# leggedrobotics/delora

Hardware: AMD Instinct MI355X
Metric: training scan-pairs/sec, KITTI 64x2048 range images (higher is better)
Workload: dtype f32; 1 GPU; KITTI-shaped 64x2048, batch=8 pairs/GPU, raw scans of ~141k points (ragged, raster order), steps rotate over 8 distinct HBM-resident batches, online normals, ResNet pose CNN (11.9M params, identity-pretrained state), Adam; BASELINE configs[1]; global_batch=8, parallelism=dp1, cnn=fp32, cnn_impl=hip trunk: fp32 MFMA, fused Winograd F(2x2,3x3) + direct implicit GEMM, channels_last=False, hip_graph=False, distinct_batches=8, priming_steps=8

## Files before the change

### delora_amd/csrc/heads.hip

```cpp
#include "common.h"

#define HD_MAXB 16

struct HeadsP {
  const float *fc_w, *fc_b;
  const float *r1_w, *r1_b;
  const float *r3_w, *r3_b;
  const float *t1_w, *t1_b;
  const float *t3_w, *t3_b;
};

__device__ __forceinline__ float hd_act(float v, int act) { return act == 1 ? dl_tanh(v) : (act == 2 ? (v < 0.f ? 0.f : v) : v); }
__device__ __forceinline__ float hd_dact(float a, int act) { return act == 1 ? 1.f - a * a : (act == 2 ? (a > 0.f ? 1.f : 0.f) : 1.f); }

__global__ __launch_bounds__(256) void k_heads_rows(const float* __restrict__ x, int B, int K, const float* __restrict__ w0, const float* __restrict__ b0,
                                                    const float* __restrict__ w1, const float* __restrict__ b1, int rows, int nmat, int act,
                                                    int KC, const float* __restrict__ pre_scale ,
                                                    float* __restrict__ y ) {
  extern __shared__ float sx[];
  const int wave = threadIdx.x >> 6, lane = threadIdx.x & 63;
  const int gr = min(blockIdx.x * 4 + wave, rows * nmat - 1);
  const int m = gr / rows, r = gr % rows;
  const float* wr = (m == 0 ? w0 : w1) + (size_t)r * K;
  float acc[HD_MAXB];
#pragma unroll
  for (int b = 0; b < HD_MAXB; ++b) acc[b] = 0.f;
  for (int k0 = 0; k0 < K; k0 += KC) {
    const int kn = min(KC, K - k0);
    __syncthreads();
    for (int q = threadIdx.x; q < B * kn; q += 256) sx[(q / kn) * KC + q % kn] = x[(size_t)(q / kn) * K + k0 + q % kn];
    __syncthreads();
#pragma unroll 8
    for (int k = lane; k < kn; k += 64) {
      const float wv = wr[k0 + k];
#pragma unroll
      for (int b = 0; b < HD_MAXB; ++b)
        if (b < B) acc[b] = fmaf(sx[b * KC + k], wv, acc[b]);
    }
  }
  if (blockIdx.x * 4 + wave >= rows * nmat) return;
  const float bias = (m == 0 ? b0 : b1)[r];
#pragma unroll
  for (int b = 0; b < HD_MAXB; ++b) {
    if (b < B) {
      const float s = wave_sum(acc[b]);
      if (lane == 0) {
        float pre = s + bias;
        if (pre_scale) pre *= pre_scale[(size_t)b * rows + r];
        y[((size_t)b * nmat + m) * rows + r] = hd_act(pre, act);
      }
    }
  }
}

__global__ __launch_bounds__(256) void k_heads_out(const float* __restrict__ a2, HeadsP p, int B, int Hd, float* __restrict__ rot_raw,
                                                   float* __restrict__ translation, float* __restrict__ rotation, float* __restrict__ norm) {
  __shared__ float raw[HD_MAXB * 7];
  __shared__ float nrm;
  const int t = threadIdx.x;
  if (t < B * 7) {
    const int b = t / 7, i = t % 7;
    const bool rot = i < 4;
    const float* w = rot ? p.r3_w + (size_t)i * Hd : p.t3_w + (size_t)(i - 4) * Hd;
    const float* a = a2 + ((size_t)b * 2 + (rot ? 0 : 1)) * Hd;
    float s = 0.f;
    for (int m = 0; m < Hd; ++m) s = fmaf(a[m], w[m], s);
    raw[t] = s + (rot ? p.r3_b[i] : p.t3_b[i - 4]);
  }
  __syncthreads();
  if (t == 0) {
    float s = 0.f;
    for (int b = 0; b < B; ++b)
      for (int i = 0; i < 4; ++i) s = fmaf(raw[b * 7 + i], raw[b * 7 + i], s);
    nrm = sqrtf(s);
    norm[0] = nrm;
  }
  __syncthreads();
  if (t < B * 7) {
    const int b = t / 7, i = t % 7;
    if (i < 4) { rot_raw[b * 4 + i] = raw[t]; rotation[b * 4 + i] = raw[t] / nrm; }
    else translation[b * 3 + (i - 4)] = raw[t];
  }
}

__global__ __launch_bounds__(256) void k_heads_out_bwd(const float* __restrict__ a2, HeadsP p, int B, int Hd, int act, const float* __restrict__ rot_raw,
                                                       const float* __restrict__ norm, const float* __restrict__ g_tr, const float* __restrict__ g_rotn,
                                                       float* __restrict__ d_r3w, float* __restrict__ d_r3b, float* __restrict__ d_t3w,
                                                       float* __restrict__ d_t3b, float* __restrict__ gh) {
  __shared__ float g[HD_MAXB * 7];
  __shared__ float dot;
  const int t = threadIdx.x;
  const float n = norm[0];
  if (t == 0) {
    float s = 0.f;
    for (int b = 0; b < B; ++b)
      for (int i = 0; i < 4; ++i) s = fmaf(g_rotn[b * 4 + i], rot_raw[b * 4 + i] / n, s);
    dot = s;
  }
  __syncthreads();
  if (t < B * 7) {
    const int b = t / 7, i = t % 7;
    g[t] = i < 4 ? (g_rotn[b * 4 + i] - (rot_raw[b * 4 + i] / n) * dot) / n : g_tr[b * 3 + (i - 4)];
  }
  __syncthreads();
  for (int q = t; q < 7 * Hd; q += blockDim.x) {
    const int i = q / Hd, m = q % Hd, head = i < 4 ? 0 : 1;
    float s = 0.f;
    for (int b = 0; b < B; ++b) s = fmaf(g[b * 7 + i], a2[((size_t)b * 2 + head) * Hd + m], s);
    if (i < 4) d_r3w[i * Hd + m] = s; else d_t3w[(i - 4) * Hd + m] = s;
  }
  if (t < 7) {
    float s = 0.f;
    for (int b = 0; b < B; ++b) s += g[b * 7 + t];
    if (t < 4) d_r3b[t] = s; else d_t3b[t - 4] = s;
  }
  for (int q = t; q < B * 2 * Hd; q += blockDim.x) {
    const int m = q % Hd, head = (q / Hd) % 2, b = q / (2 * Hd);
    float s = 0.f;
    if (head == 0) { for (int i = 0; i < 4; ++i) s = fmaf(g[b * 7 + i], p.r3_w[i * Hd + m], s); }
    else { for (int i = 0; i < 3; ++i) s = fmaf(g[b * 7 + 4 + i], p.t3_w[i * Hd + m], s); }
    gh[q] = s * hd_dact(a2[q], act);
  }
}

#define HD_HB_WAVES 8
__global__ __launch_bounds__(64 * HD_HB_WAVES) void k_heads_hidden_bwd(const float* __restrict__ a1, const float* __restrict__ gh, HeadsP p, int B, int R, int Hd,
                                                                       int act, float* __restrict__ d_r1w, float* __restrict__ d_r1b,
                                                                       float* __restrict__ d_t1w, float* __restrict__ d_t1b,
                                                                       const float* __restrict__ fc_scale , float* __restrict__ gout) {
  extern __shared__ float sgh[];
  float* red = sgh + B * 2 * Hd;
  const int lane = threadIdx.x & 63, wave = threadIdx.x >> 6;
  for (int q = threadIdx.x; q < B * 2 * Hd; q += blockDim.x) sgh[q] = gh[q];
  __syncthreads();
  if (blockIdx.x == 0)
    for (int q = threadIdx.x; q < 2 * Hd; q += blockDim.x) {
      float s = 0.f;
      for (int b = 0; b < B; ++b) s += sgh[b * 2 * Hd + q];
      if (q < Hd) d_r1b[q] = s; else d_t1b[q - Hd] = s;
    }
  const int j = blockIdx.x * 64 + lane, jj = j < R ? j : R - 1;
  float av[HD_MAXB], ga[HD_MAXB];
#pragma unroll
  for (int b = 0; b < HD_MAXB; ++b) { av[b] = b < B ? a1[(size_t)b * R + jj] : 0.f; ga[b] = 0.f; }
  const int per = (2 * Hd + HD_HB_WAVES - 1) / HD_HB_WAVES, r0 = wave * per, r1 = min(r0 + per, 2 * Hd);
#pragma unroll 5
  for (int row = r0; row < r1; ++row) {
    const bool rot = row < Hd;
    const size_t o = (size_t)(rot ? row : row - Hd) * R + jj;
    const float wv = (rot ? p.r1_w : p.t1_w)[o];
    float s = 0.f;
#pragma unroll
    for (int b = 0; b < HD_MAXB; ++b)
      if (b < B) {
        const float gv = sgh[b * 2 * Hd + row];
        ga[b] = fmaf(gv, wv, ga[b]);
        s = fmaf(gv, av[b], s);
      }
    if (j < R) (rot ? d_r1w : d_t1w)[o] = s;
  }
#pragma unroll
  for (int b = 0; b < HD_MAXB; ++b) red[(wave * HD_MAXB + b) * 64 + lane] = ga[b];
  __syncthreads();
  if (wave == 0 && j < R) {
#pragma unroll
    for (int b = 0; b < HD_MAXB; ++b)
      if (b < B) {
        float s = 0.f;
#pragma unroll
        for (int wv_ = 0; wv_ < HD_HB_WAVES; ++wv_) s += red[(wv_ * HD_MAXB + b) * 64 + lane];
        float go = s * hd_dact(av[b], act);
        if (fc_scale) go *= fc_scale[(size_t)b * R + j];
        gout[(size_t)b * R + j] = go;
      }
  }
}

#define HD_JC 40
__global__ __launch_bounds__(256) void k_heads_fc_bwd(const float* __restrict__ x, const float* __restrict__ gout, const float* __restrict__ fc_w, int B, int F,
                                                      int R, float* __restrict__ d_fcw, float* __restrict__ d_fcb, float* __restrict__ part) {
  __shared__ float sg[HD_MAXB * HD_JC];
  const int c = blockIdx.x * 256 + threadIdx.x, chunk = blockIdx.y, j0 = chunk * HD_JC;
  const int nj = min(HD_JC, R - j0);
  for (int q = threadIdx.x; q < B * nj; q += 256) sg[q] = gout[(size_t)(q / nj) * R + j0 + q % nj];
  __syncthreads();
  if (blockIdx.x == 0 && threadIdx.x < nj) {
    float s = 0.f;
    for (int b = 0; b < B; ++b) s += sg[b * nj + threadIdx.x];
    d_fcb[j0 + threadIdx.x] = s;
  }
  if (c >= F) return;
  float xv[HD_MAXB], gx[HD_MAXB];
#pragma unroll
  for (int b = 0; b < HD_MAXB; ++b) { xv[b] = b < B ? x[(size_t)b * F + c] : 0.f; gx[b] = 0.f; }
  for (int jj = 0; jj < nj; ++jj) {
    const float wv = fc_w[(size_t)(j0 + jj) * F + c];
    float s = 0.f;
#pragma unroll
    for (int b = 0; b < HD_MAXB; ++b)
      if (b < B) {
        const float gv = sg[b * nj + jj];
        gx[b] = fmaf(gv, wv, gx[b]);
        s = fmaf(gv, xv[b], s);
      }
    d_fcw[(size_t)(j0 + jj) * F + c] = s;
  }
#pragma unroll
  for (int b = 0; b < HD_MAXB; ++b)
    if (b < B) part[((size_t)chunk * B + b) * F + c] = gx[b];
}

__global__ __launch_bounds__(256) void k_heads_gx_reduce(const float* __restrict__ part, int chunks, int n, float* __restrict__ gx) {
  const int i = blockIdx.x * 256 + threadIdx.x;
  if (i >= n) return;
  float s = 0.f;
  for (int k = 0; k < chunks; ++k) s += part[(size_t)k * n + i];
  gx[i] = s;
}

static int heads_check(const char* who, const void* a, const void* b, const dl_heads_params* p, int B, int F, int R, int Hd, int act) {
  if (!a || !b || !p || !p->fc_w || !p->fc_b || !p->r1_w || !p->r1_b || !p->r3_w || !p->r3_b || !p->t1_w || !p->t1_b || !p->t3_w || !p->t3_b)
    return dl_fail(DL_ERR_INVALID_ARGUMENT, "%s: null pointer argument", who);
  if (B <= 0 || B > HD_MAXB || F <= 0 || R <= 0 || Hd <= 0 || act < 0 || act > 2)
    return dl_fail(DL_ERR_INVALID_ARGUMENT, "%s: bad size (1 <= B <= %d) or activation", who, HD_MAXB);
  return DL_OK;
}
static int heads_kc(int B, int K) {
  int kc = (48 * 1024 / 4 / B) & ~63;
  return kc >= K ? K : kc;
}
static HeadsP heads_params(const dl_heads_params* p) {
  return HeadsP{p->fc_w, p->fc_b, p->r1_w, p->r1_b, p->r3_w, p->r3_b, p->t1_w, p->t1_b, p->t3_w, p->t3_b};
}

static int heads_fwd(const char* who, const float* x, const dl_heads_params* params, int B, int F, int R, int Hd, int act, const float* fc_scale,
                     float* a1, float* a2, float* rot_raw, float* translation, float* rotation, float* norm, dl_stream stream) {
  if (int rc = heads_check(who, x, a1, params, B, F, R, Hd, act)) return rc;
  if (!a2 || !rot_raw || !translation || !rotation || !norm) return dl_fail(DL_ERR_INVALID_ARGUMENT, "%s: null output", who);
  const HeadsP p = heads_params(params);
  hipStream_t st = (hipStream_t)stream;
  const int kc_f = heads_kc(B, F), kc_r = heads_kc(B, R);
  hipLaunchKernelGGL(k_heads_rows, dim3((R + 3) / 4), dim3(256), (size_t)B * kc_f * sizeof(float), st, x, B, F, p.fc_w, p.fc_b, (const float*)nullptr, (const float*)nullptr, R, 1, act, kc_f, fc_scale, a1);
  hipLaunchKernelGGL(k_heads_rows, dim3((2 * Hd + 3) / 4), dim3(256), (size_t)B * kc_r * sizeof(float), st, (const float*)a1, B, R, p.r1_w, p.r1_b, p.t1_w, p.t1_b, Hd, 2, act, kc_r, (const float*)nullptr, a2);
  hipLaunchKernelGGL(k_heads_out, dim3(1), dim3(256), 0, st, (const float*)a2, p, B, Hd, rot_raw, translation, rotation, norm);
  return dl_check_launch(who);
}

extern "C" int dl_heads_fwd(const float* x, const dl_heads_params* params, int32_t B, int32_t F, int32_t R, int32_t Hd, int32_t act,
                            float* a1, float* a2, float* rot_raw, float* translation, float* rotation, float* norm, dl_stream stream) {
  return heads_fwd("dl_heads_fwd", x, params, B, F, R, Hd, act, nullptr, a1, a2, rot_raw, translation, rotation, norm, stream);
}

extern "C" int dl_heads_fwd_drop(const float* x, const dl_heads_params* params, int32_t B, int32_t F, int32_t R, int32_t Hd, int32_t act,
                                 const float* fc_scale, float* a1, float* a2, float* rot_raw, float* translation, float* rotation, float* norm,
                                 dl_stream stream) {
  return heads_fwd("dl_heads_fwd_drop", x, params, B, F, R, Hd, act, fc_scale, a1, a2, rot_raw, translation, rotation, norm, stream);
}

extern "C" size_t dl_heads_bwd_workspace_bytes(int32_t B, int32_t F, int32_t R, int32_t Hd) {
  if (B <= 0 || B > HD_MAXB || F <= 0 || R <= 0 || Hd <= 0) return 0;
  const size_t chunks = (size_t)(R + HD_JC - 1) / HD_JC;
  return ((size_t)B * 2 * Hd + (size_t)B * R + chunks * B * F) * sizeof(float);
}

static int heads_bwd(const char* who, const float* x, const dl_heads_params* params, int B, int F, int R, int Hd, int act, const float* fc_scale,
                     const float* a1, const float* a2, const float* rot_raw, const float* norm, const float* grad_translation,
                     const float* grad_rotation, const dl_heads_params* grads, float* grad_x, void* workspace, dl_stream stream) {
  if (int rc = heads_check(who, x, a1, params, B, F, R, Hd, act)) return rc;
  if (int rc = heads_check(who, x, a1, grads, B, F, R, Hd, act)) return rc;
  if (!a2 || !rot_raw || !norm || !grad_translation || !grad_rotation || !grad_x || !workspace)
    return dl_fail(DL_ERR_INVALID_ARGUMENT, "%s: null pointer argument", who);
  if (((size_t)B * 2 * Hd + HD_HB_WAVES * HD_MAXB * 64) * sizeof(float) > 60000) return dl_fail(DL_ERR_UNSUPPORTED, "%s: hidden layer too wide for the LDS copy", who);
  const HeadsP p = heads_params(params);
  float* gh = (float*)workspace;
  float* gout = gh + (size_t)B * 2 * Hd;
  float* part = gout + (size_t)B * R;
  const int chunks = (R + HD_JC - 1) / HD_JC;
  hipStream_t st = (hipStream_t)stream;
  hipLaunchKernelGGL(k_heads_out_bwd, dim3(1), dim3(256), 0, st, a2, p, B, Hd, act, rot_raw, norm, grad_translation, grad_rotation,
                     (float*)grads->r3_w, (float*)grads->r3_b, (float*)grads->t3_w, (float*)grads->t3_b, gh);
  hipLaunchKernelGGL(k_heads_hidden_bwd, dim3((R + 63) / 64), dim3(64 * HD_HB_WAVES), ((size_t)B * 2 * Hd + HD_HB_WAVES * HD_MAXB * 64) * sizeof(float), st, a1,
                     (const float*)gh, p, B, R, Hd, act,
                     (float*)grads->r1_w, (float*)grads->r1_b, (float*)grads->t1_w, (float*)grads->t1_b, fc_scale, gout);
  hipLaunchKernelGGL(k_heads_fc_bwd, dim3((F + 255) / 256, chunks), dim3(256), 0, st, x, (const float*)gout, p.fc_w, B, F, R, (float*)grads->fc_w,
                     (float*)grads->fc_b, part);
  hipLaunchKernelGGL(k_heads_gx_reduce, dim3((B * F + 255) / 256), dim3(256), 0, st, (const float*)part, chunks, B * F, grad_x);
  return dl_check_launch(who);
}

extern "C" int dl_heads_bwd(const float* x, const dl_heads_params* params, int32_t B, int32_t F, int32_t R, int32_t Hd, int32_t act,
                            const float* a1, const float* a2, const float* rot_raw, const float* norm, const float* grad_translation,
                            const float* grad_rotation, const dl_heads_params* grads, float* grad_x, void* workspace, dl_stream stream) {
  return heads_bwd("dl_heads_bwd", x, params, B, F, R, Hd, act, nullptr, a1, a2, rot_raw, norm, grad_translation, grad_rotation, grads, grad_x,
                   workspace, stream);
}

extern "C" int dl_heads_bwd_drop(const float* x, const dl_heads_params* params, int32_t B, int32_t F, int32_t R, int32_t Hd, int32_t act,
                                 const float* fc_scale, const float* a1, const float* a2, const float* rot_raw, const float* norm,
                                 const float* grad_translation, const float* grad_rotation, const dl_heads_params* grads, float* grad_x,
                                 void* workspace, dl_stream stream) {
  return heads_bwd("dl_heads_bwd_drop", x, params, B, F, R, Hd, act, fc_scale, a1, a2, rot_raw, norm, grad_translation, grad_rotation, grads,
                   grad_x, workspace, stream);
}

struct HeadsSingleP { const float* w[6]; const float* b[6]; };

__global__ __launch_bounds__(256) void k_heads_single_out(const float* __restrict__ a, const float* __restrict__ w, const float* __restrict__ bias, int B, int K,
                                                          float* __restrict__ rot_raw, float* __restrict__ translation, float* __restrict__ rotation,
                                                          float* __restrict__ norm) {
  __shared__ float raw[HD_MAXB * 7];
  __shared__ float nrm;
  const int t = threadIdx.x;
  if (t < B * 7) {
    const int b = t / 7, i = t % 7;
    const float* wr = w + (size_t)i * K;
    const float* ar = a + (size_t)b * K;
    float s = 0.f;
    for (int m = 0; m < K; ++m) s = fmaf(ar[m], wr[m], s);
    raw[t] = s + bias[i];
  }
  __syncthreads();
  if (t == 0) {
    float s = 0.f;
    for (int b = 0; b < B; ++b)
      for (int i = 0; i < 4; ++i) s = fmaf(raw[b * 7 + i], raw[b * 7 + i], s);
    nrm = sqrtf(s);
    norm[0] = nrm;
  }
  __syncthreads();
  if (t < B * 7) {
    const int b = t / 7, i = t % 7;
    if (i < 4) { rot_raw[b * 4 + i] = raw[t]; rotation[b * 4 + i] = raw[t] / nrm; }
    else translation[b * 3 + (i - 4)] = raw[t];
  }
}

__global__ __launch_bounds__(256) void k_heads_single_out_bwd(const float* __restrict__ a, const float* __restrict__ w, int B, int K, int act,
                                                              const float* __restrict__ rot_raw, const float* __restrict__ norm, const float* __restrict__ g_tr,
                                                              const float* __restrict__ g_rotn, float* __restrict__ d_w, float* __restrict__ d_b,
                                                              float* __restrict__ gh) {
  __shared__ float g[HD_MAXB * 7];
  __shared__ float dot;
  const int t = threadIdx.x;
  const float n = norm[0];
  if (t == 0) {
    float s = 0.f;
    for (int b = 0; b < B; ++b)
      for (int i = 0; i < 4; ++i) s = fmaf(g_rotn[b * 4 + i], rot_raw[b * 4 + i] / n, s);
    dot = s;
  }
  __syncthreads();
  if (t < B * 7) {
    const int b = t / 7, i = t % 7;
    g[t] = i < 4 ? (g_rotn[b * 4 + i] - (rot_raw[b * 4 + i] / n) * dot) / n : g_tr[b * 3 + (i - 4)];
  }
  __syncthreads();
  for (int q = t; q < 7 * K; q += blockDim.x) {
    const int i = q / K, m = q % K;
    float s = 0.f;
    for (int b = 0; b < B; ++b) s = fmaf(g[b * 7 + i], a[(size_t)b * K + m], s);
    d_w[q] = s;
  }
  if (t < 7) {
    float s = 0.f;
    for (int b = 0; b < B; ++b) s += g[b * 7 + t];
    d_b[t] = s;
  }
  for (int q = t; q < B * K; q += blockDim.x) {
    const int m = q % K, b = q / K;
    float s = 0.f;
    for (int i = 0; i < 7; ++i) s = fmaf(g[b * 7 + i], w[(size_t)i * K + m], s);
    gh[q] = s * hd_dact(a[q], act);
  }
}

__global__ __launch_bounds__(256) void k_heads_gx_reduce_act(const float* __restrict__ part, int chunks, int n, const float* __restrict__ x, int act,
                                                             const float* __restrict__ scale , float* __restrict__ gx) {
  const int i = blockIdx.x * 256 + threadIdx.x;
  if (i >= n) return;
  float s = 0.f;
  for (int k = 0; k < chunks; ++k) s += part[(size_t)k * n + i];
  float go = s * hd_dact(x[i], act);
  if (scale) go *= scale[i];
  gx[i] = go;
}

static int heads_single_check(const char* who, const dl_heads_single_params* p, int B, const int n[7], int act) {
  if (!p) return dl_fail(DL_ERR_INVALID_ARGUMENT, "%s: null pointer argument", who);
  for (int l = 0; l < 6; ++l)
    if (!p->w[l] || !p->b[l]) return dl_fail(DL_ERR_INVALID_ARGUMENT, "%s: null pointer argument", who);
  bool ok = B > 0 && B <= HD_MAXB && act >= 0 && act <= 2;
  for (int l = 0; l < 6; ++l) ok = ok && n[l] > 0 && n[l] <= (1 << 20);
  if (!ok) return dl_fail(DL_ERR_INVALID_ARGUMENT, "%s: bad size (1 <= B <= %d, every width >= 1) or activation", who, HD_MAXB);
  return DL_OK;
}
static size_t heads_single_part_floats(int B, const int n[7]) {
  size_t m = 0;
  for (int l = 0; l < 5; ++l) {
    const size_t f = (size_t)((n[l + 1] + HD_JC - 1) / HD_JC) * B * n[l];
    if (f > m) m = f;
  }
  return m;
}

extern "C" int dl_heads_single_fwd(const float* x, const dl_heads_single_params* params, int32_t B, int32_t F, int32_t R, int32_t H1, int32_t H2,
                                   int32_t H3, int32_t H4, int32_t act, const float* fc_scale, float* acts, float* rot_raw, float* translation,
                                   float* rotation, float* norm, dl_stream stream) {
  const char* who = "dl_heads_single_fwd";
  const int n[7] = {F, R, H1, H2, H3, H4, 7};
  if (!x || !acts || !rot_raw || !translation || !rotation || !norm) return dl_fail(DL_ERR_INVALID_ARGUMENT, "%s: null pointer argument", who);
  if (int rc = heads_single_check(who, params, B, n, act)) return rc;
  hipStream_t st = (hipStream_t)stream;
  const float* in = x;
  float* out = acts;
  for (int l = 0; l < 5; ++l) {
    const int K = n[l], rows = n[l + 1], kc = heads_kc(B, K);
    hipLaunchKernelGGL(k_heads_rows, dim3((rows + 3) / 4), dim3(256), (size_t)B * kc * sizeof(float), st, in, (int)B, K, params->w[l], params->b[l],
                       (const float*)nullptr, (const float*)nullptr, rows, 1, (int)act, kc, l == 0 ? fc_scale : (const float*)nullptr, out);
    in = out;
    out += (size_t)B * rows;
  }
  hipLaunchKernelGGL(k_heads_single_out, dim3(1), dim3(256), 0, st, in, params->w[5], params->b[5], (int)B, (int)H4, rot_raw, translation, rotation, norm);
  return dl_check_launch(who);
}

extern "C" size_t dl_heads_single_bwd_workspace_bytes(int32_t B, int32_t F, int32_t R, int32_t H1, int32_t H2, int32_t H3, int32_t H4) {
  const int n[7] = {F, R, H1, H2, H3, H4, 7};
  if (B <= 0 || B > HD_MAXB) return 0;
  for (int l = 0; l < 6; ++l)
    if (n[l] <= 0 || n[l] > (1 << 20)) return 0;
  return ((size_t)B * ((size_t)R + H1 + H2 + H3 + H4) + heads_single_part_floats(B, n)) * sizeof(float);
}

extern "C" int dl_heads_single_bwd(const float* x, const dl_heads_single_params* params, int32_t B, int32_t F, int32_t R, int32_t H1, int32_t H2,
                                   int32_t H3, int32_t H4, int32_t act, const float* fc_scale, const float* acts, const float* rot_raw,
                                   const float* norm, const float* grad_translation, const float* grad_rotation,
                                   const dl_heads_single_params* grads, float* grad_x, void* workspace, dl_stream stream) {
  const char* who = "dl_heads_single_bwd";
  const int n[7] = {F, R, H1, H2, H3, H4, 7};
  if (!x || !acts || !rot_raw || !norm || !grad_translation || !grad_rotation || !grad_x || !workspace)
    return dl_fail(DL_ERR_INVALID_ARGUMENT, "%s: null pointer argument", who);
  if (int rc = heads_single_check(who, params, B, n, act)) return rc;
  if (int rc = heads_single_check(who, grads, B, n, act)) return rc;
  hipStream_t st = (hipStream_t)stream;
  const float* a[5];
  float* g[5];
  {
    const float* ap = acts;
    float* gp = (float*)workspace;
    for (int l = 0; l < 5; ++l) { a[l] = ap; g[l] = gp; ap += (size_t)B * n[l + 1]; gp += (size_t)B * n[l + 1]; }
  }
  float* part = (float*)workspace + (size_t)B * ((size_t)R + H1 + H2 + H3 + H4);
  hipLaunchKernelGGL(k_heads_single_out_bwd, dim3(1), dim3(256), 0, st, a[4], params->w[5], (int)B, (int)H4, (int)act, rot_raw, norm, grad_translation,
                     grad_rotation, (float*)grads->w[5], (float*)grads->b[5], g[4]);
  for (int l = 4; l >= 0; --l) {
    const int K = n[l], M = n[l + 1], chunks = (M + HD_JC - 1) / HD_JC;
    const float* in = l ? a[l - 1] : x;
    hipLaunchKernelGGL(k_heads_fc_bwd, dim3((K + 255) / 256, chunks), dim3(256), 0, st, in, (const float*)g[l], params->w[l], (int)B, K, M,
                       (float*)grads->w[l], (float*)grads->b[l], part);
    if (l)
      hipLaunchKernelGGL(k_heads_gx_reduce_act, dim3((B * K + 255) / 256), dim3(256), 0, st, (const float*)part, chunks, B * K, in, (int)act,
                         l == 1 ? fc_scale : (const float*)nullptr, g[l - 1]);
    else
      hipLaunchKernelGGL(k_heads_gx_reduce, dim3((B * K + 255) / 256), dim3(256), 0, st, (const float*)part, chunks, B * K, grad_x);
  }
  return dl_check_launch(who);
}
```

Measured before the change: 698.1 scan-pairs/s.

## Speed up FC heads kernels with prefetching, vector staging and split backward

Reworks several pose-head kernels. The row GEMV now prefetches weights in registers and stages inputs with float4 copies. The output kernels stage activations and weights in shared memory. The FC backward splits columns across four waves, with weights staged in LDS and the batch split per wave. The chunk-sum reduction is unrolled by eight. These target latency-bound loads in small head kernels, at the cost of more registers and LDS use, while the head cost is small next to the CNN trunk.

```diff
diff --git a/delora_amd/csrc/heads.hip b/delora_amd/csrc/heads.hip
--- a/delora_amd/csrc/heads.hip
+++ b/delora_amd/csrc/heads.hip
@@ -13,6 +13,7 @@
 __device__ __forceinline__ float hd_act(float v, int act) { return act == 1 ? dl_tanh(v) : (act == 2 ? (v < 0.f ? 0.f : v) : v); }
 __device__ __forceinline__ float hd_dact(float a, int act) { return act == 1 ? 1.f - a * a : (act == 2 ? (a > 0.f ? 1.f : 0.f) : 1.f); }
 
+#define HD_RW 8
 __global__ __launch_bounds__(256) void k_heads_rows(const float* __restrict__ x, int B, int K, const float* __restrict__ w0, const float* __restrict__ b0,
                                                     const float* __restrict__ w1, const float* __restrict__ b1, int rows, int nmat, int act,
                                                     int KC, const float* __restrict__ pre_scale ,
@@ -25,17 +26,42 @@
   float acc[HD_MAXB];
 #pragma unroll
   for (int b = 0; b < HD_MAXB; ++b) acc[b] = 0.f;
+  float wv[HD_RW];
+  {
+    const int kn = min(KC, K);
+#pragma unroll
+    for (int i = 0; i < HD_RW; ++i) wv[i] = lane + 64 * i < kn ? wr[lane + 64 * i] : 0.f;
+  }
+  const bool vec = !(K & 3) && !(KC & 3) && !((size_t)x & 15);
   for (int k0 = 0; k0 < K; k0 += KC) {
     const int kn = min(KC, K - k0);
     __syncthreads();
-    for (int q = threadIdx.x; q < B * kn; q += 256) sx[(q / kn) * KC + q % kn] = x[(size_t)(q / kn) * K + k0 + q % kn];
+    if (vec) {
+      const int kn4 = kn >> 2;
+#pragma unroll 4
+      for (int b = 0; b < B; ++b)
+        for (int q = threadIdx.x; q < kn4; q += 256)
+          reinterpret_cast<float4*>(sx + (size_t)b * KC)[q] = reinterpret_cast<const float4*>(x + (size_t)b * K + k0)[q];
+    } else {
+#pragma unroll 4
+      for (int b = 0; b < B; ++b)
+        for (int q = threadIdx.x; q < kn; q += 256) sx[b * KC + q] = x[(size_t)b * K + k0 + q];
+    }
     __syncthreads();
-#pragma unroll 8
-    for (int k = lane; k < kn; k += 64) {
-      const float wv = wr[k0 + k];
-#pragma unroll
-      for (int b = 0; b < HD_MAXB; ++b)
-        if (b < B) acc[b] = fmaf(sx[b * KC + k], wv, acc[b]);
+    for (int kb = lane; kb < kn; kb += 64 * HD_RW) {
+      if (k0 | (kb - lane)) {
+#pragma unroll
+        for (int i = 0; i < HD_RW; ++i) wv[i] = kb + 64 * i < kn ? wr[k0 + kb + 64 * i] : 0.f;
+      }
+#pragma unroll
+      for (int i = 0; i < HD_RW; ++i) {
+        const int k = kb + 64 * i;
+        if (k < kn) {
+#pragma unroll
+          for (int b = 0; b < HD_MAXB; ++b)
+            if (b < B) acc[b] = fmaf(sx[b * KC + k], wv[i], acc[b]);
+        }
+      }
     }
   }
   if (blockIdx.x * 4 + wave >= rows * nmat) return;
@@ -53,16 +79,41 @@
   }
 }
 
+#define HD_STAGE_MAX_FLOATS (56 * 1024 / 4)
+__device__ __forceinline__ void hd_stage(float* __restrict__ dst, const float* __restrict__ src, int n) {
+  constexpr int THREADS = 256;
+  for (int q0 = threadIdx.x; q0 < n; q0 += 8 * THREADS) {
+    float v[8];
+#pragma unroll
+    for (int u = 0; u < 8; ++u) v[u] = q0 + u * THREADS < n ? src[q0 + u * THREADS] : 0.f;
+#pragma unroll
+    for (int u = 0; u < 8; ++u)
+      if (q0 + u * THREADS < n) dst[q0 + u * THREADS] = v[u];
+  }
+}
+
+template <bool STAGE>
 __global__ __launch_bounds__(256) void k_heads_out(const float* __restrict__ a2, HeadsP p, int B, int Hd, float* __restrict__ rot_raw,
                                                    float* __restrict__ translation, float* __restrict__ rotation, float* __restrict__ norm) {
+  extern __shared__ float sh_out[];
   __shared__ float raw[HD_MAXB * 7];
   __shared__ float nrm;
   const int t = threadIdx.x;
+  const float* __restrict__ sa = a2;
+  const float* __restrict__ swr = p.r3_w;
+  const float* __restrict__ swt = p.t3_w;
+  if constexpr (STAGE) {
+    hd_stage(sh_out, a2, B * 2 * Hd);
+    hd_stage(sh_out + B * 2 * Hd, p.r3_w, 4 * Hd);
+    hd_stage(sh_out + B * 2 * Hd + 4 * Hd, p.t3_w, 3 * Hd);
+    sa = sh_out; swr = sh_out + B * 2 * Hd; swt = swr + 4 * Hd;
+    __syncthreads();
+  }
   if (t < B * 7) {
     const int b = t / 7, i = t % 7;
     const bool rot = i < 4;
-    const float* w = rot ? p.r3_w + (size_t)i * Hd : p.t3_w + (size_t)(i - 4) * Hd;
-    const float* a = a2 + ((size_t)b * 2 + (rot ? 0 : 1)) * Hd;
+    const float* w = rot ? swr + (size_t)i * Hd : swt + (size_t)(i - 4) * Hd;
+    const float* a = sa + ((size_t)b * 2 + (rot ? 0 : 1)) * Hd;
     float s = 0.f;
     for (int m = 0; m < Hd; ++m) s = fmaf(a[m], w[m], s);
     raw[t] = s + (rot ? p.r3_b[i] : p.t3_b[i - 4]);
@@ -177,45 +228,75 @@
 }
 
 #define HD_JC 40
-__global__ __launch_bounds__(256) void k_heads_fc_bwd(const float* __restrict__ x, const float* __restrict__ gout, const float* __restrict__ fc_w, int B, int F,
-                                                      int R, float* __restrict__ d_fcw, float* __restrict__ d_fcb, float* __restrict__ part) {
+#define HD_FB_COLS 64
+#define HD_FB_GROUPS 4
+#define HD_FB_ROWS (HD_JC / HD_FB_GROUPS)
+#define HD_FB_BS (HD_MAXB / HD_FB_GROUPS)
+__global__ __launch_bounds__(HD_FB_COLS * HD_FB_GROUPS) void k_heads_fc_bwd(const float* __restrict__ x, const float* __restrict__ gout, const float* __restrict__ fc_w,
+                                                                            int B, int F, int R, float* __restrict__ d_fcw, float* __restrict__ d_fcb,
+                                                                            float* __restrict__ part) {
   __shared__ float sg[HD_MAXB * HD_JC];
-  const int c = blockIdx.x * 256 + threadIdx.x, chunk = blockIdx.y, j0 = chunk * HD_JC;
+  __shared__ float sw[HD_JC][HD_FB_COLS];
+  const int lane = threadIdx.x & 63, g = threadIdx.x >> 6;
+  const int c = blockIdx.x * HD_FB_COLS + lane, chunk = blockIdx.y, j0 = chunk * HD_JC;
   const int nj = min(HD_JC, R - j0);
-  for (int q = threadIdx.x; q < B * nj; q += 256) sg[q] = gout[(size_t)(q / nj) * R + j0 + q % nj];
-  __syncthreads();
-  if (blockIdx.x == 0 && threadIdx.x < nj) {
+  const int cc = c < F ? c : F - 1;
+  float wl[HD_FB_ROWS], xv[HD_MAXB], gx[HD_FB_BS];
+#pragma unroll
+  for (int i = 0; i < HD_FB_ROWS; ++i) wl[i] = g * HD_FB_ROWS + i < nj ? fc_w[(size_t)(j0 + g * HD_FB_ROWS + i) * F + cc] : 0.f;
+#pragma unroll
+  for (int b = 0; b < HD_MAXB; ++b) xv[b] = b < B ? x[(size_t)b * F + cc] : 0.f;
+  if (lane < nj)
+    for (int b = g; b < B; b += HD_FB_GROUPS) sg[b * nj + lane] = gout[(size_t)b * R + j0 + lane];
+#pragma unroll
+  for (int i = 0; i < HD_FB_ROWS; ++i) sw[g * HD_FB_ROWS + i][lane] = wl[i];
+  __syncthreads();
+  if (blockIdx.x == 0 && (int)threadIdx.x < nj) {
     float s = 0.f;
     for (int b = 0; b < B; ++b) s += sg[b * nj + threadIdx.x];
     d_fcb[j0 + threadIdx.x] = s;
   }
+#pragma unroll
+  for (int bi = 0; bi < HD_FB_BS; ++bi) gx[bi] = 0.f;
+#pragma unroll 4
+  for (int jj = 0; jj < nj; ++jj) {
+    const float wv = sw[jj][lane];
+#pragma unroll
+    for (int bi = 0; bi < HD_FB_BS; ++bi)
+      if (g + HD_FB_GROUPS * bi < B) gx[bi] = fmaf(sg[(g + HD_FB_GROUPS * bi) * nj + jj], wv, gx[bi]);
+  }
   if (c >= F) return;
-  float xv[HD_MAXB], gx[HD_MAXB];
-#pragma unroll
-  for (int b = 0; b < HD_MAXB; ++b) { xv[b] = b < B ? x[(size_t)b * F + c] : 0.f; gx[b] = 0.f; }
-  for (int jj = 0; jj < nj; ++jj) {
-    const float wv = fc_w[(size_t)(j0 + jj) * F + c];
+#pragma unroll
+  for (int bi = 0; bi < HD_FB_BS; ++bi)
+    if (g + HD_FB_GROUPS * bi < B) part[((size_t)chunk * B + g + HD_FB_GROUPS * bi) * F + c] = gx[bi];
+  for (int jj = g * HD_FB_ROWS; jj < min((g + 1) * HD_FB_ROWS, nj); ++jj) {
     float s = 0.f;
 #pragma unroll
     for (int b = 0; b < HD_MAXB; ++b)
-      if (b < B) {
-        const float gv = sg[b * nj + jj];
-        gx[b] = fmaf(gv, wv, gx[b]);
-        s = fmaf(gv, xv[b], s);
-      }
+      if (b < B) s = fmaf(sg[b * nj + jj], xv[b], s);
     d_fcw[(size_t)(j0 + jj) * F + c] = s;
   }
-#pragma unroll
-  for (int b = 0; b < HD_MAXB; ++b)
-    if (b < B) part[((size_t)chunk * B + b) * F + c] = gx[b];
+}
+static_assert(HD_JC <= 64 && HD_JC % HD_FB_GROUPS == 0 && HD_MAXB % HD_FB_GROUPS == 0, "k_heads_fc_bwd: a lane per chunk row, equal shares per wave");
+
+__device__ __forceinline__ float hd_chunk_sum(const float* __restrict__ part, int chunks, int n, int i) {
+  float s = 0.f;
+  int k = 0;
+  for (; k + 8 <= chunks; k += 8) {
+    float v[8];
+#pragma unroll
+    for (int u = 0; u < 8; ++u) v[u] = part[(size_t)(k + u) * n + i];
+#pragma unroll
+    for (int u = 0; u < 8; ++u) s += v[u];
+  }
+  for (; k < chunks; ++k) s += part[(size_t)k * n + i];
+  return s;
 }
 
 __global__ __launch_bounds__(256) void k_heads_gx_reduce(const float* __restrict__ part, int chunks, int n, float* __restrict__ gx) {
   const int i = blockIdx.x * 256 + threadIdx.x;
   if (i >= n) return;
-  float s = 0.f;
-  for (int k = 0; k < chunks; ++k) s += part[(size_t)k * n + i];
-  gx[i] = s;
+  gx[i] = hd_chunk_sum(part, chunks, n, i);
 }
 
 static int heads_check(const char* who, const void* a, const void* b, const dl_heads_params* p, int B, int F, int R, int Hd, int act) {
@@ -242,7 +323,11 @@
   const int kc_f = heads_kc(B, F), kc_r = heads_kc(B, R);
   hipLaunchKernelGGL(k_heads_rows, dim3((R + 3) / 4), dim3(256), (size_t)B * kc_f * sizeof(float), st, x, B, F, p.fc_w, p.fc_b, (const float*)nullptr, (const float*)nullptr, R, 1, act, kc_f, fc_scale, a1);
   hipLaunchKernelGGL(k_heads_rows, dim3((2 * Hd + 3) / 4), dim3(256), (size_t)B * kc_r * sizeof(float), st, (const float*)a1, B, R, p.r1_w, p.r1_b, p.t1_w, p.t1_b, Hd, 2, act, kc_r, (const float*)nullptr, a2);
-  hipLaunchKernelGGL(k_heads_out, dim3(1), dim3(256), 0, st, (const float*)a2, p, B, Hd, rot_raw, translation, rotation, norm);
+  const size_t stage = ((size_t)B * 2 + 7) * Hd;
+  if (stage <= HD_STAGE_MAX_FLOATS)
+    hipLaunchKernelGGL(k_heads_out<true>, dim3(1), dim3(256), stage * sizeof(float), st, (const float*)a2, p, B, Hd, rot_raw, translation, rotation, norm);
+  else
+    hipLaunchKernelGGL(k_heads_out<false>, dim3(1), dim3(256), 0, st, (const float*)a2, p, B, Hd, rot_raw, translation, rotation, norm);
   return dl_check_launch(who);
 }
 
@@ -282,7 +367,7 @@
   hipLaunchKernelGGL(k_heads_hidden_bwd, dim3((R + 63) / 64), dim3(64 * HD_HB_WAVES), ((size_t)B * 2 * Hd + HD_HB_WAVES * HD_MAXB * 64) * sizeof(float), st, a1,
                      (const float*)gh, p, B, R, Hd, act,
                      (float*)grads->r1_w, (float*)grads->r1_b, (float*)grads->t1_w, (float*)grads->t1_b, fc_scale, gout);
-  hipLaunchKernelGGL(k_heads_fc_bwd, dim3((F + 255) / 256, chunks), dim3(256), 0, st, x, (const float*)gout, p.fc_w, B, F, R, (float*)grads->fc_w,
+  hipLaunchKernelGGL(k_heads_fc_bwd, dim3((F + HD_FB_COLS - 1) / HD_FB_COLS, chunks), dim3(HD_FB_COLS * HD_FB_GROUPS), 0, st, x, (const float*)gout, p.fc_w, B, F, R, (float*)grads->fc_w,
                      (float*)grads->fc_b, part);
   hipLaunchKernelGGL(k_heads_gx_reduce, dim3((B * F + 255) / 256), dim3(256), 0, st, (const float*)part, chunks, B * F, grad_x);
   return dl_check_launch(who);
@@ -305,16 +390,26 @@
 
 struct HeadsSingleP { const float* w[6]; const float* b[6]; };
 
+template <bool STAGE>
 __global__ __launch_bounds__(256) void k_heads_single_out(const float* __restrict__ a, const float* __restrict__ w, const float* __restrict__ bias, int B, int K,
                                                           float* __restrict__ rot_raw, float* __restrict__ translation, float* __restrict__ rotation,
                                                           float* __restrict__ norm) {
+  extern __shared__ float sh_out[];
   __shared__ float raw[HD_MAXB * 7];
   __shared__ float nrm;
   const int t = threadIdx.x;
+  const float* __restrict__ sa = a;
+  const float* __restrict__ sw = w;
+  if constexpr (STAGE) {
+    hd_stage(sh_out, a, B * K);
+    hd_stage(sh_out + B * K, w, 7 * K);
+    sa = sh_out; sw = sh_out + B * K;
+    __syncthreads();
+  }
   if (t < B * 7) {
     const int b = t / 7, i = t % 7;
-    const float* wr = w + (size_t)i * K;
-    const float* ar = a + (size_t)b * K;
+    const float* wr = sw + (size_t)i * K;
+    const float* ar = sa + (size_t)b * K;
     float s = 0.f;
     for (int m = 0; m < K; ++m) s = fmaf(ar[m], wr[m], s);
     raw[t] = s + bias[i];
@@ -378,8 +473,7 @@
                                                              const float* __restrict__ scale , float* __restrict__ gx) {
   const int i = blockIdx.x * 256 + threadIdx.x;
   if (i >= n) return;
-  float s = 0.f;
-  for (int k = 0; k < chunks; ++k) s += part[(size_t)k * n + i];
+  const float s = hd_chunk_sum(part, chunks, n, i);
   float go = s * hd_dact(x[i], act);
   if (scale) go *= scale[i];
   gx[i] = go;
@@ -420,7 +514,12 @@
     in = out;
     out += (size_t)B * rows;
   }
-  hipLaunchKernelGGL(k_heads_single_out, dim3(1), dim3(256), 0, st, in, params->w[5], params->b[5], (int)B, (int)H4, rot_raw, translation, rotation, norm);
+  const size_t stage = ((size_t)B + 7) * H4;
+  if (stage <= HD_STAGE_MAX_FLOATS)
+    hipLaunchKernelGGL(k_heads_single_out<true>, dim3(1), dim3(256), stage * sizeof(float), st, in, params->w[5], params->b[5], (int)B, (int)H4, rot_raw, translation,
+                       rotation, norm);
+  else
+    hipLaunchKernelGGL(k_heads_single_out<false>, dim3(1), dim3(256), 0, st, in, params->w[5], params->b[5], (int)B, (int)H4, rot_raw, translation, rotation, norm);
   return dl_check_launch(who);
 }
 
@@ -456,7 +555,7 @@
   for (int l = 4; l >= 0; --l) {
     const int K = n[l], M = n[l + 1], chunks = (M + HD_JC - 1) / HD_JC;
     const float* in = l ? a[l - 1] : x;
-    hipLaunchKernelGGL(k_heads_fc_bwd, dim3((K + 255) / 256, chunks), dim3(256), 0, st, in, (const float*)g[l], params->w[l], (int)B, K, M,
+    hipLaunchKernelGGL(k_heads_fc_bwd, dim3((K + HD_FB_COLS - 1) / HD_FB_COLS, chunks), dim3(HD_FB_COLS * HD_FB_GROUPS), 0, st, in, (const float*)g[l], params->w[l], (int)B, K, M,
                        (float*)grads->w[l], (float*)grads->b[l], part);
     if (l)
       hipLaunchKernelGGL(k_heads_gx_reduce_act, dim3((B * K + 255) / 256), dim3(256), 0, st, (const float*)part, chunks, B * K, in, (int)act,
```

New measurement: 701.1 scan-pairs/s, median of 6. Within noise of the previous version (+0.4%).
